# ilpoviertola/V-AURA

Measured on AMD Instinct MI355X. Metric: audio codec tokens/sec (whole node), 2.56 s clips, higher is better.
Workload: dtype f16x2-split(22b)/f32-acc

## Files before the change

### vaura_amd/csrc/step.hip

```cpp
#include "common.h"
#include "gemv3_kernel.h"

__global__ void token_table_kernel(const float* __restrict__ tok_emb, const float* __restrict__ proj_w,
                                   const float* __restrict__ proj_b, float* __restrict__ table, int K, int vocab1,
                                   int cdim, int tok_dim) {
  const int64_t i = (int64_t)blockIdx.x * blockDim.x + threadIdx.x;
  const int64_t total = (int64_t)K * vocab1 * tok_dim;
  if (i >= total) return;
  const int c = (int)(i % tok_dim);
  const int tok = (int)((i / tok_dim) % vocab1);
  const int k = (int)(i / ((int64_t)tok_dim * vocab1));
  const float* e = tok_emb + ((size_t)k * vocab1 + tok) * cdim;
  const float* wr = proj_w + ((size_t)k * tok_dim + c) * cdim;
  float z = 0.f;
  for (int j = 0; j < cdim; ++j) z = fmaf(wr[j], e[j], z);
  table[i] = z + proj_b[(size_t)k * tok_dim + c];
}

__global__ __launch_bounds__(64) void embed_kernel(
    const int32_t* __restrict__ seq, const int32_t* __restrict__ state, const float* __restrict__ cond_proj,
    const float* __restrict__ empty_video, const float* __restrict__ table, float* __restrict__ h,
    uint16_t* __restrict__ hsplit, const float* __restrict__ gain, float* __restrict__ ss, int B, int K, int S, int Tv,
    int tpf, int vocab1, int cond_dim, int tok_dim, int pos_host, int rows16) {
  const int row = blockIdx.x;
  const int cq = blockIdx.y * 64 + threadIdx.x;
  const int b = row % B;
  const int pos = pos_host >= 0 ? pos_host + (int)blockIdx.z : state[0];
  const int vrow = (int)blockIdx.z * rows16 + row;
  const int D = cond_dim + tok_dim;
  const int frame = pos / tpf;
  f32x4 o;
  if (cq < cond_dim / 4) {
    if (frame < Tv)
      o = reinterpret_cast<const f32x4*>(cond_proj)[packed_quad(row * Tv + frame, cq, cond_dim)];
    else
      o = reinterpret_cast<const f32x4*>(empty_video)[cq];
  } else {
    const int c0 = (cq - cond_dim / 4) * 4;
    o = f32x4{0.f, 0.f, 0.f, 0.f};
    int tok[16];
#pragma unroll
    for (int k = 0; k < 16; ++k) tok[k] = (k < K) ? seq[((size_t)b * K + k) * S + pos] : 0;
    f32x4 e[16];
#pragma unroll
    for (int k = 0; k < 16; ++k)
      if (k < K) e[k] = *reinterpret_cast<const f32x4*>(table + ((size_t)k * vocab1 + tok[k]) * tok_dim + c0);
#pragma unroll
    for (int k = 0; k < 16; ++k)
      if (k < K) o += e[k];
  }
  va_st16(reinterpret_cast<f32x4*>(h) + packed_quad(vrow, cq, D), o);
  if (hsplit) {
    float s = ((o[0] * o[0] + o[1] * o[1]) + o[2] * o[2]) + o[3] * o[3];
    s += __shfl_xor(s, 1, 64);
    s += __shfl_xor(s, 2, 64);
    if ((threadIdx.x & 3) == 0) va_st4(ss + ((size_t)(vrow >> 4) * (D / 16) + (cq >> 2)) * 16 + (vrow & 15), s);
    const f32x4 u = o * *reinterpret_cast<const f32x4*>(gain + cq * 4);
    store_split4(hsplit, vrow, cq * 4, D, u);
  }
}

int va_launch_embed(const vaura_decoder* d, int pos_host, int n_pos, hipStream_t s) {
  const vaura_dims& m = d->dims;
  const int D = m.cond_dim + m.tok_dim;
  if (!d->tok_table || (D % 256)) return VAURA_ERR_SHAPE;
  const bool split = d->wdtype == VAURA_W_H1 || d->wdtype == VAURA_W_H2 || va_is_fp8(d->wdtype);
  if (split && (!d->ws_h_split || !d->ws_ss || !d->first_norm)) return VAURA_ERR_ARG;
  VA_LAUNCH(embed_kernel, dim3(d->rows, D / 256, n_pos), dim3(64), 0, s, d->seq, d->state, d->cond_proj, d->empty_video,
            d->tok_table, d->ws_h, split ? d->ws_h_split : nullptr, d->first_norm, d->ws_ss, d->batch, m.n_codebooks,
            d->seq_len, d->n_cond_tokens, m.tokens_per_frame, m.vocab + 1, m.cond_dim, m.tok_dim, pos_host,
            (d->rows + 15) / 16 * 16);
  return 0;
}

extern "C" int vaura_build_token_table(const float* tok_emb, const float* proj_w, const float* proj_b, float* table, int K,
                                       int vocab1, int cdim, int tok_dim, vaura_stream_t s) {
  if (!tok_emb || !proj_w || !proj_b || !table || K <= 0) return VAURA_ERR_ARG;
  const int64_t total = (int64_t)K * vocab1 * tok_dim;
  VA_LAUNCH(token_table_kernel, dim3((unsigned)((total + 255) / 256)), dim3(256), 0, as_stream(s), tok_emb, proj_w, proj_b,
            table, K, vocab1, cdim, tok_dim);
  return 0;
}

__device__ __forceinline__ void philox4x32_10(uint32_t c0, uint32_t c1, uint32_t c2, uint32_t c3, uint32_t k0,
                                              uint32_t k1, uint32_t out[4]) {
#pragma unroll
  for (int r = 0; r < 10; ++r) {
    const uint64_t p0 = (uint64_t)0xD2511F53u * c0, p1 = (uint64_t)0xCD9E8D57u * c2;
    const uint32_t n0 = (uint32_t)(p1 >> 32) ^ c1 ^ k0, n1 = (uint32_t)p1;
    const uint32_t n2 = (uint32_t)(p0 >> 32) ^ c3 ^ k1, n3 = (uint32_t)p0;
    c0 = n0; c1 = n1; c2 = n2; c3 = n3;
    k0 += 0x9E3779B9u; k1 += 0xBB67AE85u;
  }
  out[0] = c0; out[1] = c1; out[2] = c2; out[3] = c3;
}

struct SampleArgs {
  const float* logits;
  const float* noise;
  const int32_t* state;
  int32_t* state_rw;
  int32_t* tokens_out;
  int32_t* seq;
  int B, K, V, T, S;
  int use_sampling, top_k, probs_in;
  float temp, top_p, cfg_scale;
  float tie_eps;
  uint64_t seed, clip_base;
  long long step_host;
};

#define SMP_THREADS 256

__device__ __forceinline__ void block_argmax(float v, int i, float* sv, int* si, float& bv, int& bi) {
#pragma unroll
  for (int o = 32; o > 0; o >>= 1) {
    const float ov = __shfl_xor(v, o, 64);
    const int oi = __shfl_xor(i, o, 64);
    if (ov > v || (ov == v && oi < i)) { v = ov; i = oi; }
  }
  __syncthreads();
  if ((threadIdx.x & 63) == 0) { sv[threadIdx.x >> 6] = v; si[threadIdx.x >> 6] = i; }
  __syncthreads();
  bv = sv[0]; bi = si[0];
#pragma unroll
  for (int w = 1; w < SMP_THREADS / 64; ++w)
    if (sv[w] > bv || (sv[w] == bv && si[w] < bi)) { bv = sv[w]; bi = si[w]; }
}

__device__ __forceinline__ float block_sum(float v, float* sv) {
  v = wave_sum(v);
  __syncthreads();
  if ((threadIdx.x & 63) == 0) sv[threadIdx.x >> 6] = v;
  __syncthreads();
  return ((sv[0] + sv[1]) + sv[2]) + sv[3];
}
__device__ __forceinline__ float block_max(float v, float* sv) {
  v = wave_max(v);
  __syncthreads();
  if ((threadIdx.x & 63) == 0) sv[threadIdx.x >> 6] = v;
  __syncthreads();
  return fmaxf(fmaxf(sv[0], sv[1]), fmaxf(sv[2], sv[3]));
}
__device__ __forceinline__ void block_max2(float& a, float& b, float* sv) {
  a = wave_max(a);
  b = wave_max(b);
  __syncthreads();
  if ((threadIdx.x & 63) == 0) { sv[threadIdx.x >> 6] = a; sv[4 + (threadIdx.x >> 6)] = b; }
  __syncthreads();
  a = fmaxf(fmaxf(sv[0], sv[1]), fmaxf(sv[2], sv[3]));
  b = fmaxf(fmaxf(sv[4], sv[5]), fmaxf(sv[6], sv[7]));
}
__device__ __forceinline__ void block_tie4(float& m0, float& m1, int& c0, int& c1, float* sv, int* si) {
  m0 = wave_max(m0);
  m1 = wave_max(m1);
#pragma unroll
  for (int o = 32; o > 0; o >>= 1) { c0 += __shfl_xor(c0, o, 64); c1 += __shfl_xor(c1, o, 64); }
  __syncthreads();
  if ((threadIdx.x & 63) == 0) {
    const int wv = threadIdx.x >> 6;
    sv[wv] = m0; sv[4 + wv] = m1; si[wv] = c0; si[4 + wv] = c1;
  }
  __syncthreads();
  m0 = fmaxf(fmaxf(sv[0], sv[1]), fmaxf(sv[2], sv[3]));
  m1 = fmaxf(fmaxf(sv[4], sv[5]), fmaxf(sv[6], sv[7]));
  c0 = si[0] + si[1] + si[2] + si[3];
  c1 = si[4] + si[5] + si[6] + si[7];
}
__device__ __forceinline__ int block_count(int v, int* si) {
#pragma unroll
  for (int o = 32; o > 0; o >>= 1) v += __shfl_xor(v, o, 64);
  __syncthreads();
  if ((threadIdx.x & 63) == 0) si[threadIdx.x >> 6] = v;
  __syncthreads();
  return si[0] + si[1] + si[2] + si[3];
}

__global__ __launch_bounds__(SMP_THREADS) void sample_kernel(const float* __restrict__ logits_q, const int32_t* __restrict__ state_q,
                                                             SampleArgs a) {
  a.logits = logits_q;
  a.state = state_q;
  __shared__ float sv[8];
  __shared__ int si[8];
  __shared__ float sp[1024];
  __shared__ int sidx[1024];
  __shared__ float skeep[1024];
  __shared__ uint32_t hist[256];
  __shared__ uint32_t s_sel[2];
  const int k = blockIdx.x, b = blockIdx.y, tid = threadIdx.x;
  const int pos = a.state ? a.state[0] : 0;
  const long long step = a.state ? (long long)a.state[2] : a.step_host;
  const int V = a.V;

  const f32x4 lc = *reinterpret_cast<const f32x4*>(a.logits + ((size_t)b * a.K + k) * V + 4 * tid);
  float x[4] = {lc[0], lc[1], lc[2], lc[3]};
  float amax = fmaxf(fmaxf(fabsf(lc[0]), fabsf(lc[1])), fmaxf(fabsf(lc[2]), fabsf(lc[3])));
  if (a.cfg_scale > 1.0f) {
    const f32x4 lu = *reinterpret_cast<const f32x4*>(a.logits + ((size_t)(a.B + b) * a.K + k) * V + 4 * tid);
    amax = fmaxf(amax, fmaxf(fmaxf(fabsf(lu[0]), fabsf(lu[1])), fmaxf(fabsf(lu[2]), fabsf(lu[3]))));
#pragma unroll
    for (int j = 0; j < 4; ++j) x[j] = lu[j] + (x[j] - lu[j]) * a.cfg_scale;
  }
  bool near_tie = false;
  float tie_delta = 0.f;
  const bool tie_on = a.tie_eps > 0.f && !a.probs_in;
  const float tie_mix = a.tie_eps * (a.cfg_scale > 1.0f ? 2.f * a.cfg_scale - 1.f : 1.f);
  if (tie_on && !(a.use_sampling && a.temp > 0.0f)) tie_delta = tie_mix * block_max(amax, sv);
  if (!(fabsf(x[0]) < INFINITY && fabsf(x[1]) < INFINITY && fabsf(x[2]) < INFINITY && fabsf(x[3]) < INFINITY)) {
    if (a.state_rw) __hip_atomic_fetch_or(&a.state_rw[4], VAURA_STATUS_NONFINITE_LOGITS, __ATOMIC_RELAXED, __HIP_MEMORY_SCOPE_AGENT);
#pragma unroll
    for (int j = 0; j < 4; ++j) x[j] = fabsf(x[j]) < INFINITY ? x[j] : 0.f;
  }

  int token;
  if (!(a.use_sampling && a.temp > 0.0f)) {
    float bv = x[0]; int bi = 4 * tid;
#pragma unroll
    for (int j = 1; j < 4; ++j) if (x[j] > bv) { bv = x[j]; bi = 4 * tid + j; }
    float rv; int ri;
    block_argmax(bv, bi, sv, si, rv, ri);
    token = ri;
    if (tie_delta > 0.f) {
      float second = -INFINITY;
#pragma unroll
      for (int j = 0; j < 4; ++j) if (4 * tid + j != ri) second = fmaxf(second, x[j]);
      second = block_max(second, sv);
      near_tie = (rv - second) < 2.f * tie_delta;
    }
  } else {
    float p[4];
    if (a.probs_in) {
#pragma unroll
      for (int j = 0; j < 4; ++j) p[j] = x[j];
    } else {
#pragma unroll
      for (int j = 0; j < 4; ++j) x[j] = x[j] / a.temp;
      float mx = fmaxf(fmaxf(x[0], x[1]), fmaxf(x[2], x[3]));
      if (tie_on) {
        block_max2(mx, amax, sv);
        tie_delta = tie_mix * amax;
      } else {
        mx = block_max(mx, sv);
      }
#pragma unroll
      for (int j = 0; j < 4; ++j) p[j] = expf(x[j] - mx);
      const float den = block_sum((p[0] + p[1]) + (p[2] + p[3]), sv);
#pragma unroll
      for (int j = 0; j < 4; ++j) p[j] = p[j] / den;
    }

    float q[4];
    if (a.noise) {
      const f32x4 nz = *reinterpret_cast<const f32x4*>(a.noise + (((size_t)step * a.B + b) * a.K + k) * V + 4 * tid);
      q[0] = nz[0]; q[1] = nz[1]; q[2] = nz[2]; q[3] = nz[3];
    } else {
      uint32_t r[4];
      const uint64_t clip = a.clip_base + (uint64_t)b;
      philox4x32_10((uint32_t)tid, (uint32_t)step, (uint32_t)(clip * (uint64_t)a.K + k), (uint32_t)((clip * a.K + k) >> 32),
                    (uint32_t)a.seed, (uint32_t)(a.seed >> 32), r);
#pragma unroll
      for (int j = 0; j < 4; ++j) q[j] = -logf(((float)r[j] + 0.5f) * 2.3283064365386963e-10f);
    }

    if (a.top_p > 0.0f) {
      float sp_r[4];
      int id_r[4];
#pragma unroll
      for (int j = 0; j < 4; ++j) { sp_r[j] = p[j]; id_r[j] = 4 * tid + j; }
      auto cmpx = [&](int j, float py, int idy, int st, int sz) {
        const int i = 4 * tid + j;
        const bool lower = (i & st) == 0;
        const bool desc = ((i & ~st) & sz) == 0;
        const bool x_first = (sp_r[j] > py) || (sp_r[j] == py && id_r[j] < idy);
        const bool keep_x = (lower == desc) ? x_first : !x_first;
        if (!keep_x) { sp_r[j] = py; id_r[j] = idy; }
      };
      for (int sz = 2; sz <= 1024; sz <<= 1) {
        for (int st = sz >> 1; st > 0; st >>= 1) {
          if (st == 1) {
            const float py[4] = {sp_r[1], sp_r[0], sp_r[3], sp_r[2]};
            const int iy[4] = {id_r[1], id_r[0], id_r[3], id_r[2]};
#pragma unroll
            for (int j = 0; j < 4; ++j) cmpx(j, py[j], iy[j], 1, sz);
          } else if (st == 2) {
            const float py[4] = {sp_r[2], sp_r[3], sp_r[0], sp_r[1]};
            const int iy[4] = {id_r[2], id_r[3], id_r[0], id_r[1]};
#pragma unroll
            for (int j = 0; j < 4; ++j) cmpx(j, py[j], iy[j], 2, sz);
          } else if (st < 256) {
            float py[4]; int iy[4];
#pragma unroll
            for (int j = 0; j < 4; ++j) { py[j] = __shfl_xor(sp_r[j], st >> 2, 64); iy[j] = __shfl_xor(id_r[j], st >> 2, 64); }
            const bool want_first = (((4 * tid) & st) == 0) == ((((4 * tid) & ~st) & sz) == 0);
#pragma unroll
            for (int j = 0; j < 4; ++j) {
              const bool x_first = (sp_r[j] > py[j]) || (sp_r[j] == py[j] && id_r[j] < iy[j]);
              if (x_first != want_first) { sp_r[j] = py[j]; id_r[j] = iy[j]; }
            }
          } else {
            __syncthreads();
#pragma unroll
            for (int j = 0; j < 4; ++j) { sp[4 * tid + j] = sp_r[j]; sidx[4 * tid + j] = id_r[j]; }
            __syncthreads();
            float py[4]; int iy[4];
#pragma unroll
            for (int j = 0; j < 4; ++j) { py[j] = sp[(4 * tid + j) ^ st]; iy[j] = sidx[(4 * tid + j) ^ st]; }
#pragma unroll
            for (int j = 0; j < 4; ++j) cmpx(j, py[j], iy[j], st, sz);
          }
        }
      }
      __syncthreads();
#pragma unroll
      for (int j = 0; j < 4; ++j) { sp[4 * tid + j] = sp_r[j]; sidx[4 * tid + j] = id_r[j]; }
      __syncthreads();
      if (tid < 64) {
        float v[16], keep[16];
#pragma unroll
        for (int j = 0; j < 4; ++j) {
          const f32x4 x = *reinterpret_cast<const f32x4*>(sp + 16 * tid + 4 * j);
          v[4 * j] = x[0]; v[4 * j + 1] = x[1]; v[4 * j + 2] = x[2]; v[4 * j + 3] = x[3];
        }
        float carry = 0.f;
        for (int l = 0; l < 64; ++l) {
          float cs = carry;
#pragma unroll
          for (int j = 0; j < 16; ++j) {
            cs += v[j];
            if (tid == l) keep[j] = (cs - v[j] > a.top_p) ? 0.f : 1.f;
          }
          carry = __builtin_bit_cast(float, __builtin_amdgcn_readlane(__builtin_bit_cast(int, cs), l));
        }
#pragma unroll
        for (int j = 0; j < 4; ++j)
          *reinterpret_cast<f32x4*>(skeep + 16 * tid + 4 * j) = f32x4{keep[4 * j], keep[4 * j + 1], keep[4 * j + 2], keep[4 * j + 3]};
      }
      __syncthreads();
      float ps[4];
#pragma unroll
      for (int j = 0; j < 4; ++j) ps[j] = sp[4 * tid + j] * skeep[4 * tid + j];
      const float den2 = block_sum((ps[0] + ps[1]) + (ps[2] + ps[3]), sv);
      float bv = -1.f; int bi = 0x7fffffff;
#pragma unroll
      for (int j = 0; j < 4; ++j) {
        const float r = (ps[j] / den2) / q[j];
        if (r > bv) { bv = r; bi = 4 * tid + j; }
      }
      float rv; int ri;
      block_argmax(bv, bi, sv, si, rv, ri);
      token = sidx[ri];
      if (tie_delta > 0.f) {
        float second = -1.f;
#pragma unroll
        for (int j = 0; j < 4; ++j) if (4 * tid + j != ri) second = fmaxf(second, (ps[j] / den2) / q[j]);
        second = block_max(second, sv);
        near_tie = (rv - second) < rv * (2.f * tie_delta / a.temp);
      }
    } else {
      const float p_raw[4] = {p[0], p[1], p[2], p[3]};
      float thr_keep = 0.f, den_keep = 1.f;
      if (a.top_k > 0) {
        const int kk = a.top_k < V ? a.top_k : V;
        uint32_t key[4];
#pragma unroll
        for (int j = 0; j < 4; ++j) key[j] = __builtin_bit_cast(uint32_t, p[j]);
        uint32_t thr = 0;
        int need = kk;
#pragma unroll 1
        for (int pass = 0; pass < 4; ++pass) {
          const int shift = 24 - 8 * pass;
          hist[tid] = 0;
          __syncthreads();
#pragma unroll
          for (int j = 0; j < 4; ++j)
            if (pass == 0 || (key[j] >> (shift + 8)) == (thr >> (shift + 8))) atomicAdd(&hist[(key[j] >> shift) & 255u], 1u);
          __syncthreads();
          const int mine = (int)hist[255 - tid];
          int scan = mine;
#pragma unroll
          for (int o = 1; o < 64; o <<= 1) {
            const int up = __shfl_up(scan, o, 64);
            if ((tid & 63) >= o) scan += up;
          }
          if ((tid & 63) == 63) si[tid >> 6] = scan;
          __syncthreads();
          for (int w2 = 0; w2 < (tid >> 6); ++w2) scan += si[w2];
          if (scan >= need && scan - mine < need) {
            s_sel[0] = thr | ((uint32_t)(255 - tid) << shift);
            s_sel[1] = (uint32_t)(need - (scan - mine));
          }
          __syncthreads();
          thr = s_sel[0];
          need = (int)s_sel[1];
        }
        const float thrf = __builtin_bit_cast(float, thr);
        thr_keep = thrf;
#pragma unroll
        for (int j = 0; j < 4; ++j) p[j] = p[j] * (p[j] >= thrf ? 1.0f : 0.0f);
        const float den2 = block_sum((p[0] + p[1]) + (p[2] + p[3]), sv);
        den_keep = den2;
#pragma unroll
        for (int j = 0; j < 4; ++j) p[j] = p[j] / den2;
      }
      float bv = -1.f; int bi = 0x7fffffff;
#pragma unroll
      for (int j = 0; j < 4; ++j) {
        const float r = p[j] / q[j];
        if (r > bv) { bv = r; bi = 4 * tid + j; }
      }
      float rv; int ri;
      block_argmax(bv, bi, sv, si, rv, ri);
      token = ri;
      if (tie_delta > 0.f) {
        const float band = 2.f * tie_delta / a.temp;
        float second = -1.f, cand = -1.f;
        int nbelow = 0, wedge = 0;
#pragma unroll
        for (int j = 0; j < 4; ++j) {
          const int i = 4 * tid + j;
          if (i != ri) second = fmaxf(second, p[j] / q[j]);
          if (thr_keep > 0.f) {
            if (p_raw[j] < thr_keep && p_raw[j] >= thr_keep * (1.f - band)) { ++nbelow; cand = fmaxf(cand, (p_raw[j] / den_keep) / q[j]); }
            if (i == ri && p_raw[j] <= thr_keep * (1.f + band)) wedge = 1;
          }
        }
        block_tie4(second, cand, nbelow, wedge, sv, si);
        near_tie = (rv - second) < rv * band;
        if (thr_keep > 0.f && (cand >= rv * (1.f - band) || (nbelow > 0 && wedge > 0))) near_tie = true;
      }
    }
  }

  if (tid == 0) {
    if (a.tokens_out) a.tokens_out[b * a.K + k] = token;
    if (a.seq) {
      const int offset = pos + 1;
      const int t = offset - 1 - k;
      const int tok = (t >= 0 && t < a.T) ? token : V;
      if (offset < a.S) {
        int32_t* slot = a.seq + ((size_t)b * a.K + k) * a.S + offset;
        if (*slot == -1) {
          *slot = tok;
          if (near_tie && t >= 0 && t < a.T && a.state_rw) {
            __hip_atomic_fetch_or(&a.state_rw[4], VAURA_STATUS_NEAR_TIE, __ATOMIC_RELAXED, __HIP_MEMORY_SCOPE_AGENT);
            __hip_atomic_fetch_add(&a.state_rw[6], 1, __ATOMIC_RELAXED, __HIP_MEMORY_SCOPE_AGENT);
            int expect = 0;
            (void)__hip_atomic_compare_exchange_strong(&a.state_rw[7], &expect, (int)step + 1, __ATOMIC_RELAXED, __ATOMIC_RELAXED, __HIP_MEMORY_SCOPE_AGENT);
          }
        }
      }
    }
    if (a.state_rw) {
      const int arrived = __hip_atomic_fetch_add(&a.state_rw[1], 1, __ATOMIC_RELAXED, __HIP_MEMORY_SCOPE_AGENT);
      if (arrived == (int)(gridDim.x * gridDim.y) - 1) {
        __hip_atomic_store(&a.state_rw[1], 0, __ATOMIC_RELAXED, __HIP_MEMORY_SCOPE_AGENT);
        a.state_rw[0] = pos + 1;
        a.state_rw[2] = (int)step + 1;
        a.state_rw[5] = a.state_rw[5] + 1;
      }
    }
  }
}

int va_launch_sample(const float* logits, int B, int K, int vocab, const vaura_sampling* sp, const float* noise,
                     int , const int32_t* state, int64_t step_host, int32_t* tokens_out,
                     int32_t* seq, int T, int S, int32_t* state_rw, hipStream_t s) {
  if (!logits || !sp || B <= 0 || K <= 0) return VAURA_ERR_ARG;
  if (vocab != 1024) return VAURA_ERR_SHAPE;
  SampleArgs a;
  a.logits = logits; a.noise = noise; a.state = state; a.state_rw = state_rw; a.tokens_out = tokens_out; a.seq = seq;
  a.B = B; a.K = K; a.V = vocab; a.T = T; a.S = S;
  a.use_sampling = sp->use_sampling; a.top_k = sp->top_k; a.temp = sp->temp; a.top_p = sp->top_p;
  a.cfg_scale = sp->input_is_probs ? 1.0f : sp->cfg_scale; a.seed = sp->seed; a.clip_base = sp->clip_base; a.step_host = step_host;
  a.probs_in = sp->input_is_probs;
  a.tie_eps = sp->tie_eps > 0.f ? sp->tie_eps : 0.f;
  VA_LAUNCH(sample_kernel, dim3(K, B), dim3(SMP_THREADS), 0, s, a.logits, a.state, a);
  return 0;
}

__global__ void advance_kernel(int32_t* state, int set_to) {
  if (threadIdx.x == 0 && blockIdx.x == 0) {
    state[0] = set_to >= 0 ? set_to : state[0] + 1;
    state[5] = state[5] + 1;
  }
}
int va_launch_advance(int32_t* state, int set_to, hipStream_t s) {
  VA_LAUNCH(advance_kernel, dim3(1), dim3(64), 0, s, state, set_to);
  return 0;
}

__global__ void pattern_build_kernel(const int32_t* __restrict__ codes, int32_t* __restrict__ seq, int B, int K, int T,
                                     int special) {
  const int S = T + K;
  const int64_t i = (int64_t)blockIdx.x * blockDim.x + threadIdx.x;
  if (i >= (int64_t)B * K * S) return;
  const int s = (int)(i % S), q = (int)((i / S) % K), b = (int)(i / ((int64_t)S * K));
  const int t = s - 1 - q;
  seq[i] = (t >= 0 && t < T) ? codes[((size_t)b * K + q) * T + t] : special;
}
__global__ void pattern_revert_kernel(const int32_t* __restrict__ seq, int32_t* __restrict__ codes, int B, int K, int T,
                                      int S, int fill) {
  const int64_t i = (int64_t)blockIdx.x * blockDim.x + threadIdx.x;
  if (i >= (int64_t)B * K * T) return;
  const int t = (int)(i % T), q = (int)((i / T) % K), b = (int)(i / ((int64_t)T * K));
  const int s = t + 1 + q;
  codes[i] = (s < S) ? seq[((size_t)b * K + q) * S + s] : fill;
}

extern "C" {

int vaura_pattern_build(const int32_t* codes, int32_t* seq, int B, int K, int T, int special, vaura_stream_t s) {
  if (!codes || !seq || B <= 0 || K <= 0 || T <= 0) return VAURA_ERR_ARG;
  const int64_t n = (int64_t)B * K * (T + K);
  VA_LAUNCH(pattern_build_kernel, dim3((unsigned)((n + 255) / 256)), dim3(256), 0, as_stream(s), codes, seq, B, K, T, special);
  return 0;
}

int vaura_pattern_revert(const int32_t* seq, int32_t* codes, int B, int K, int T, int S, int fill, vaura_stream_t s) {
  if (!codes || !seq || B <= 0 || K <= 0 || T <= 0 || S <= 0) return VAURA_ERR_ARG;
  const int64_t n = (int64_t)B * K * T;
  VA_LAUNCH(pattern_revert_kernel, dim3((unsigned)((n + 255) / 256)), dim3(256), 0, as_stream(s), seq, codes, B, K, T, S, fill);
  return 0;
}

int vaura_sample(const float* logits, int B, int K, int vocab, const vaura_sampling* sp, const float* noise,
                 int64_t step, int32_t* tokens_out, vaura_stream_t s) {
  if (!tokens_out) return VAURA_ERR_ARG;
  return va_launch_sample(logits, B, K, vocab, sp, noise, B * K, nullptr, step, tokens_out, nullptr, 0, 0, nullptr, as_stream(s));
}

}
```

Baseline: 74780.

## Add fast sampling kernel with radix-select top-k and register-resident logits

Adds a specialized sampling kernel for the vocab-1024 case where each thread holds four logits in registers. It uses wave-shuffle argmax and reductions, and a 4-pass 8-bit radix histogram select for the top-k threshold in place of the generic sampler's path. Dispatch keeps the original kernel for top-p sampling or when a debug flag is set, and uses the fast kernel otherwise. This cuts the per-step sampling latency inside the decode loop, at the cost of a second code path whose tie detection and top-k semantics must match the original.

Result: no change. 74870, median of 6 (+0.1%).

```diff
diff --git a/vaura_amd/csrc/step.hip b/vaura_amd/csrc/step.hip
--- a/vaura_amd/csrc/step.hip
+++ b/vaura_amd/csrc/step.hip
@@ -462,6 +462,290 @@
   }
 }
 
+__device__ __forceinline__ void argmax_step(float& v, int& i, float ov, int oi) {
+  if (ov > v || (ov == v && oi < i)) { v = ov; i = oi; }
+}
+__device__ __forceinline__ void wave_argmax(float& v, int& i) {
+#pragma unroll
+  for (int o = 32; o > 0; o >>= 1) {
+    const float ov = __shfl_xor(v, o, 64);
+    const int oi = __shfl_xor(i, o, 64);
+    argmax_step(v, i, ov, oi);
+  }
+}
+__device__ __forceinline__ int wave_count(int c) {
+#pragma unroll
+  for (int o = 32; o > 0; o >>= 1) c += __shfl_xor(c, o, 64);
+  return c;
+}
+__device__ __forceinline__ void radix_pick(const uint32_t* __restrict__ h, int shift, uint32_t& thr, int& need) {
+  const int lane = threadIdx.x & 63;
+  const uint4 hv = *reinterpret_cast<const uint4*>(h + 252 - 4 * lane);
+  const int c0 = (int)hv.w, c1 = c0 + (int)hv.z, c2 = c1 + (int)hv.y, c3 = c2 + (int)hv.x;
+  int scan = c3;
+#pragma unroll
+  for (int o = 1; o < 64; o <<= 1) {
+    const int up = __shfl_up(scan, o, 64);
+    if (lane >= o) scan += up;
+  }
+  const int ex = scan - c3;
+  const bool here = ex < need && ex + c3 >= need;
+  const unsigned long long m = __ballot(here);
+  const int src = __ffsll((long long)m) - 1;
+  const int j = ex + c0 >= need ? 0 : ex + c1 >= need ? 1 : ex + c2 >= need ? 2 : 3;
+  const int above = j == 0 ? ex : j == 1 ? ex + c0 : j == 2 ? ex + c1 : ex + c2;
+  const int pick = __shfl(255 - 4 * lane - j, src, 64);
+  const int nabove = __shfl(above, src, 64);
+  thr |= (uint32_t)pick << shift;
+  need -= nabove;
+}
+
+__global__ __launch_bounds__(SMP_THREADS) void sample_fast_kernel(const float* __restrict__ logits_q, const int32_t* __restrict__ state_q,
+                                                                  SampleArgs a) {
+  a.logits = logits_q;
+  a.state = state_q;
+  __shared__ float s_m[8];
+  __shared__ float s_s[4];
+  __shared__ float s_s2[4];
+  __shared__ float s_av[4], s_a2[4], s_ac[4];
+  __shared__ int s_ai[4], s_an[4], s_aw[4];
+  __shared__ __attribute__((aligned(16))) uint32_t hist[4][256];
+  const int k = blockIdx.x, b = blockIdx.y, tid = threadIdx.x, wv = tid >> 6;
+  const int pos = a.state ? a.state[0] : 0;
+  const long long step = a.state ? (long long)a.state[2] : a.step_host;
+  const int V = a.V;
+  const bool sampled = a.use_sampling && a.temp > 0.0f;
+  const bool topk = sampled && a.top_k > 0;
+
+  const f32x4 lc = *reinterpret_cast<const f32x4*>(a.logits + ((size_t)b * a.K + k) * V + 4 * tid);
+  f32x4 lu = lc;
+  if (a.cfg_scale > 1.0f) lu = *reinterpret_cast<const f32x4*>(a.logits + ((size_t)(a.B + b) * a.K + k) * V + 4 * tid);
+  const int offset = pos + 1;
+  int32_t* slot = nullptr;
+  int32_t slot_v = 0;
+  if (tid == 0 && a.seq && offset < a.S) {
+    slot = a.seq + ((size_t)b * a.K + k) * a.S + offset;
+    slot_v = *slot;
+  }
+  if (topk) {
+#pragma unroll
+    for (int h = 0; h < 4; ++h) hist[h][tid] = 0u;
+  }
+  float q[4] = {1.f, 1.f, 1.f, 1.f};
+  if (sampled) {
+    if (a.noise) {
+      const f32x4 nz = *reinterpret_cast<const f32x4*>(a.noise + (((size_t)step * a.B + b) * a.K + k) * V + 4 * tid);
+      q[0] = nz[0]; q[1] = nz[1]; q[2] = nz[2]; q[3] = nz[3];
+    } else {
+      uint32_t r[4];
+      const uint64_t clip = a.clip_base + (uint64_t)b;
+      philox4x32_10((uint32_t)tid, (uint32_t)step, (uint32_t)(clip * (uint64_t)a.K + k), (uint32_t)((clip * a.K + k) >> 32),
+                    (uint32_t)a.seed, (uint32_t)(a.seed >> 32), r);
+#pragma unroll
+      for (int j = 0; j < 4; ++j) q[j] = -logf(((float)r[j] + 0.5f) * 2.3283064365386963e-10f);
+    }
+  }
+
+  float x[4] = {lc[0], lc[1], lc[2], lc[3]};
+  float amax = fmaxf(fmaxf(fabsf(lc[0]), fabsf(lc[1])), fmaxf(fabsf(lc[2]), fabsf(lc[3])));
+  if (a.cfg_scale > 1.0f) {
+    amax = fmaxf(amax, fmaxf(fmaxf(fabsf(lu[0]), fabsf(lu[1])), fmaxf(fabsf(lu[2]), fabsf(lu[3]))));
+#pragma unroll
+    for (int j = 0; j < 4; ++j) x[j] = lu[j] + (x[j] - lu[j]) * a.cfg_scale;
+  }
+  bool near_tie = false;
+  float tie_delta = 0.f;
+  const bool tie_on = a.tie_eps > 0.f && !a.probs_in;
+  const float tie_mix = a.tie_eps * (a.cfg_scale > 1.0f ? 2.f * a.cfg_scale - 1.f : 1.f);
+  if (!(fabsf(x[0]) < INFINITY && fabsf(x[1]) < INFINITY && fabsf(x[2]) < INFINITY && fabsf(x[3]) < INFINITY)) {
+    if (a.state_rw) __hip_atomic_fetch_or(&a.state_rw[4], VAURA_STATUS_NONFINITE_LOGITS, __ATOMIC_RELAXED, __HIP_MEMORY_SCOPE_AGENT);
+#pragma unroll
+    for (int j = 0; j < 4; ++j) x[j] = fabsf(x[j]) < INFINITY ? x[j] : 0.f;
+  }
+
+  int token;
+  if (!sampled) {
+    float bv = x[0]; int bi = 4 * tid;
+#pragma unroll
+    for (int j = 1; j < 4; ++j) if (x[j] > bv) { bv = x[j]; bi = 4 * tid + j; }
+    float v = bv; int i = bi;
+    wave_argmax(v, i);
+    float sec = 0.f;
+    if (tie_on) {
+      float own2 = -INFINITY;
+#pragma unroll
+      for (int j = 0; j < 4; ++j) if (4 * tid + j != bi) own2 = fmaxf(own2, x[j]);
+      sec = wave_max(bi == i ? own2 : bv);
+      amax = wave_max(amax);
+    }
+    if ((tid & 63) == 0) { s_av[wv] = v; s_ai[wv] = i; s_a2[wv] = sec; s_m[wv] = amax; }
+    __syncthreads();
+    float rv = s_av[0]; int ri = s_ai[0], rw = 0;
+#pragma unroll
+    for (int w = 1; w < SMP_THREADS / 64; ++w)
+      if (s_av[w] > rv || (s_av[w] == rv && s_ai[w] < ri)) { rv = s_av[w]; ri = s_ai[w]; rw = w; }
+    token = ri;
+    if (tie_on) {
+      tie_delta = tie_mix * fmaxf(fmaxf(s_m[0], s_m[1]), fmaxf(s_m[2], s_m[3]));
+      if (tie_delta > 0.f) {
+        float second = -INFINITY;
+#pragma unroll
+        for (int w = 0; w < SMP_THREADS / 64; ++w) second = fmaxf(second, w == rw ? s_a2[w] : s_av[w]);
+        near_tie = (rv - second) < 2.f * tie_delta;
+      }
+    }
+  } else {
+    float p[4];
+    float den = 1.f;
+    if (a.probs_in) {
+#pragma unroll
+      for (int j = 0; j < 4; ++j) p[j] = x[j];
+      if (topk) {
+        __syncthreads();
+#pragma unroll
+        for (int j = 0; j < 4; ++j) atomicAdd(&hist[0][__builtin_bit_cast(uint32_t, p[j]) >> 24], 1u);
+        __syncthreads();
+      }
+    } else {
+      if (a.temp != 1.0f) {
+#pragma unroll
+        for (int j = 0; j < 4; ++j) x[j] = x[j] / a.temp;
+      }
+      float mx = fmaxf(fmaxf(x[0], x[1]), fmaxf(x[2], x[3]));
+      mx = wave_max(mx);
+      if (tie_on) amax = wave_max(amax);
+      if ((tid & 63) == 0) { s_m[wv] = mx; s_m[4 + wv] = amax; }
+      __syncthreads();
+      mx = fmaxf(fmaxf(s_m[0], s_m[1]), fmaxf(s_m[2], s_m[3]));
+      if (tie_on) tie_delta = tie_mix * fmaxf(fmaxf(s_m[4], s_m[5]), fmaxf(s_m[6], s_m[7]));
+#pragma unroll
+      for (int j = 0; j < 4; ++j) p[j] = expf(x[j] - mx);
+      if (topk) {
+#pragma unroll
+        for (int j = 0; j < 4; ++j) atomicAdd(&hist[0][__builtin_bit_cast(uint32_t, p[j]) >> 24], 1u);
+      }
+      const float ws = wave_sum((p[0] + p[1]) + (p[2] + p[3]));
+      if ((tid & 63) == 0) s_s[wv] = ws;
+      __syncthreads();
+      den = ((s_s[0] + s_s[1]) + s_s[2]) + s_s[3];
+      if (!topk) {
+#pragma unroll
+        for (int j = 0; j < 4; ++j) p[j] = p[j] / den;
+      }
+    }
+
+    float p_raw[4] = {p[0], p[1], p[2], p[3]};
+    float thr_keep = 0.f, den_keep = 1.f;
+    if (topk) {
+      uint32_t key[4];
+#pragma unroll
+      for (int j = 0; j < 4; ++j) key[j] = __builtin_bit_cast(uint32_t, p[j]);
+      uint32_t thr = 0;
+      int need = a.top_k < V ? a.top_k : V;
+      radix_pick(hist[0], 24, thr, need);
+#pragma unroll 1
+      for (int pass = 1; pass < 4; ++pass) {
+        const int shift = 24 - 8 * pass;
+#pragma unroll
+        for (int j = 0; j < 4; ++j)
+          if ((key[j] >> (shift + 8)) == (thr >> (shift + 8))) atomicAdd(&hist[pass][(key[j] >> shift) & 255u], 1u);
+        __syncthreads();
+        radix_pick(hist[pass], shift, thr, need);
+      }
+      float thrf = __builtin_bit_cast(float, thr);
+      if (!a.probs_in) {
+        thrf = thrf / den;
+#pragma unroll
+        for (int j = 0; j < 4; ++j) { p[j] = p[j] / den; p_raw[j] = p[j]; }
+      }
+      thr_keep = thrf;
+#pragma unroll
+      for (int j = 0; j < 4; ++j) p[j] = p[j] * (p[j] >= thrf ? 1.0f : 0.0f);
+      const float ws2 = wave_sum((p[0] + p[1]) + (p[2] + p[3]));
+      if ((tid & 63) == 0) s_s2[wv] = ws2;
+      __syncthreads();
+      const float den2 = ((s_s2[0] + s_s2[1]) + s_s2[2]) + s_s2[3];
+      den_keep = den2;
+#pragma unroll
+      for (int j = 0; j < 4; ++j) p[j] = p[j] / den2;
+    }
+
+    const float band = 2.f * tie_delta / a.temp;
+    float bv = -1.f; int bi = 0x7fffffff;
+    float r[4];
+#pragma unroll
+    for (int j = 0; j < 4; ++j) {
+      r[j] = p[j] / q[j];
+      if (r[j] > bv) { bv = r[j]; bi = 4 * tid + j; }
+    }
+    float v = bv; int i = bi;
+    wave_argmax(v, i);
+    float sec = -1.f, cand = -1.f;
+    int nbelow = 0, wedge = 0;
+    if (tie_delta > 0.f) {
+      float own2 = -1.f;
+#pragma unroll
+      for (int j = 0; j < 4; ++j) {
+        if (4 * tid + j != bi) own2 = fmaxf(own2, r[j]);
+        if (thr_keep > 0.f) {
+          if (p_raw[j] < thr_keep && p_raw[j] >= thr_keep * (1.f - band)) { ++nbelow; cand = fmaxf(cand, (p_raw[j] / den_keep) / q[j]); }
+          if (4 * tid + j == i && p_raw[j] <= thr_keep * (1.f + band)) wedge = 1;
+        }
+      }
+      sec = wave_max(bi == i ? own2 : bv);
+      if (thr_keep > 0.f) {
+        cand = wave_max(cand);
+        nbelow = wave_count(nbelow);
+        wedge = wave_count(wedge);
+      }
+    }
+    if ((tid & 63) == 0) { s_av[wv] = v; s_ai[wv] = i; s_a2[wv] = sec; s_ac[wv] = cand; s_an[wv] = nbelow; s_aw[wv] = wedge; }
+    __syncthreads();
+    float rv = s_av[0]; int ri = s_ai[0], rw = 0;
+#pragma unroll
+    for (int w = 1; w < SMP_THREADS / 64; ++w)
+      if (s_av[w] > rv || (s_av[w] == rv && s_ai[w] < ri)) { rv = s_av[w]; ri = s_ai[w]; rw = w; }
+    token = ri;
+    if (tie_delta > 0.f) {
+      float second = -1.f, cnd = -1.f;
+      int nb = 0;
+#pragma unroll
+      for (int w = 0; w < SMP_THREADS / 64; ++w) {
+        second = fmaxf(second, w == rw ? s_a2[w] : s_av[w]);
+        cnd = fmaxf(cnd, s_ac[w]);
+        nb += s_an[w];
+      }
+      near_tie = (rv - second) < rv * band;
+      if (thr_keep > 0.f && (cnd >= rv * (1.f - band) || (nb > 0 && s_aw[rw] > 0))) near_tie = true;
+    }
+  }
+  if (tid == 0) {
+    if (a.tokens_out) a.tokens_out[b * a.K + k] = token;
+    if (slot) {
+      const int t = offset - 1 - k;
+      const int tok = (t >= 0 && t < a.T) ? token : V;
+      if (slot_v == -1) {
+        *slot = tok;
+        if (near_tie && t >= 0 && t < a.T && a.state_rw) {
+          __hip_atomic_fetch_or(&a.state_rw[4], VAURA_STATUS_NEAR_TIE, __ATOMIC_RELAXED, __HIP_MEMORY_SCOPE_AGENT);
+          __hip_atomic_fetch_add(&a.state_rw[6], 1, __ATOMIC_RELAXED, __HIP_MEMORY_SCOPE_AGENT);
+          int expect = 0;
+          (void)__hip_atomic_compare_exchange_strong(&a.state_rw[7], &expect, (int)step + 1, __ATOMIC_RELAXED, __ATOMIC_RELAXED, __HIP_MEMORY_SCOPE_AGENT);
+        }
+      }
+    }
+    if (a.state_rw) {
+      const int arrived = __hip_atomic_fetch_add(&a.state_rw[1], 1, __ATOMIC_RELAXED, __HIP_MEMORY_SCOPE_AGENT);
+      if (arrived == (int)(gridDim.x * gridDim.y) - 1) {
+        __hip_atomic_store(&a.state_rw[1], 0, __ATOMIC_RELAXED, __HIP_MEMORY_SCOPE_AGENT);
+        a.state_rw[0] = pos + 1;
+        a.state_rw[2] = (int)step + 1;
+        a.state_rw[5] = a.state_rw[5] + 1;
+      }
+    }
+  }
+}
+
 int va_launch_sample(const float* logits, int B, int K, int vocab, const vaura_sampling* sp, const float* noise,
                      int , const int32_t* state, int64_t step_host, int32_t* tokens_out,
                      int32_t* seq, int T, int S, int32_t* state_rw, hipStream_t s) {
@@ -474,7 +758,13 @@
   a.cfg_scale = sp->input_is_probs ? 1.0f : sp->cfg_scale; a.seed = sp->seed; a.clip_base = sp->clip_base; a.step_host = step_host;
   a.probs_in = sp->input_is_probs;
   a.tie_eps = sp->tie_eps > 0.f ? sp->tie_eps : 0.f;
-  VA_LAUNCH(sample_kernel, dim3(K, B), dim3(SMP_THREADS), 0, s, a.logits, a.state, a);
+  if (a.top_p > 0.0f && a.use_sampling && a.temp > 0.0f) {
+    VA_LAUNCH(sample_kernel, dim3(K, B), dim3(SMP_THREADS), 0, s, a.logits, a.state, a);
+  } else if (va_debug_flags2_get() & 0x1000000u) {
+    VA_LAUNCH(sample_kernel, dim3(K, B), dim3(SMP_THREADS), 0, s, a.logits, a.state, a);
+  } else {
+    VA_LAUNCH(sample_fast_kernel, dim3(K, B), dim3(SMP_THREADS), 0, s, a.logits, a.state, a);
+  }
   return 0;
 }
 
```
